# yeyupiaoling/PPASR

Measured on AMD Instinct MI355X. Metric: audio-seconds/s (RTF^-1) Conformer-streaming fbank, batch32 per GPU, ctc_greedy, higher is better.
Workload: dtype f32

## Files before the change

ppasr_amd/csrc/front_fused.hip:

```cpp
#include "conformer_kernels.h"
#include "launch.h"

namespace ppasr {

template <int MT>
__global__ __launch_bounds__(kThreads) void k_conv12(const float* __restrict__ feats, FrontW fw, float* __restrict__ out,
                                                     int T, int F, int Tp, int F2, int M, int m0, PadSkip ps,
                                                     const int* __restrict__ tile_tab) {
  constexpr int BM = 32 * MT, KC = 128, LD = KC + 4, G = KC / 8, NL = 2 * MT, STEP = G / NL, N_CHUNKS = 18;
  int r0 = m0 + blockIdx.x * BM, Mlim = M;
  if (tile_tab) {
    const int t = blockIdx.x, nb = tile_tab[0];
    const int* pre = tile_tab + 1;
    if (t >= pre[nb]) return;
    int lo = 0, hi = nb;
    while (hi - lo > 1) {
      const int mid = (lo + hi) >> 1;
      if (pre[mid] <= t) lo = mid;
      else hi = mid;
    }
    const int S = ps.Tp * ps.unit;
    r0 = lo * S + (t - pre[lo]) * BM;
    Mlim = min(M, (lo + 1) * S);
  } else if (pad_block_skippable(ps, r0, BM, M)) {
    return;
  }
  extern __shared__ __attribute__((aligned(16))) float smem[];
  float* xs = smem + 2 * BM * LD;
  const int tid = threadIdx.x, lane = lane_id(), wave = wave_id();
  constexpr int tile_stride = N_CHUNKS * G * 64;
  const f32x4* wbase = fw.conv2_w + (size_t)wave * tile_stride;
  BRing<1> ring;
  ring_prime(ring, wbase, 0);
  const int bt0 = r0 / F2, nbt = (min(r0 + BM, Mlim) - 1) / F2 - bt0 + 1;
  for (int idx = tid; idx < nbt * 7 * F; idx += kThreads) {
    const int p = idx / F, f = idx - p * F;
    const int btl = p / 7, fr = p - 7 * btl;
    const int bt = bt0 + btl, b = bt / Tp, tp = bt - b * Tp;
    const int t = min(4 * tp + fr, T - 1);
    xs[idx] = (feats[((size_t)b * T + t) * F + f] - fw.cmvn_mean[f]) * fw.cmvn_istd[f];
  }
  const int c4 = tid & 31, rbase = tid >> 5;
  uint32_t pb[MT];
#pragma unroll
  for (int i = 0; i < NL; ++i) {
    const int m = r0 + rbase + 16 * i;
    const int bt = m / F2, f2 = m - bt * F2;
    const uint32_t v = m < Mlim ? (uint32_t)((bt - bt0) * 7 * F + 4 * f2) : 0xffffu;
    pb[i >> 1] = (i & 1) ? (pb[i >> 1] | (v << 16)) : v;
  }
  auto pbase = [&](int i) { return (int)((i & 1) ? (pb[i >> 1] >> 16) : (pb[i >> 1] & 0xffffu)); };
  const int lds_off0 = rbase * LD + 4 * c4;
  f32x4 wv[9], bv;
  float xv[9];
  auto load_w = [&](int kc) {
    const int c = (kc & 1) * 128 + 4 * c4;
#pragma unroll
    for (int j = 0; j < 9; ++j) wv[j] = *reinterpret_cast<const f32x4*>(fw.conv1_w + j * 256 + c);
    bv = *reinterpret_cast<const f32x4*>(fw.conv1_b + c);
  };
  auto read_x = [&](int i, int toff) {
    const int o = pbase(i);
    const float* p = xs + (o == 0xffff ? 0 : o) + toff;
#pragma unroll
    for (int ii = 0; ii < 3; ++ii)
#pragma unroll
      for (int jj = 0; jj < 3; ++jj) xv[ii * 3 + jj] = p[ii * F + jj];
  };
  auto fma_row = [&](int i, float* buf) {
    f32x4 a = {0.f, 0.f, 0.f, 0.f};
#pragma unroll
    for (int j = 0; j < 9; ++j)
#pragma unroll
      for (int e = 0; e < 4; ++e) a[e] = fmaf(wv[j][e], xv[j], a[e]);
    a += bv;
#pragma unroll
    for (int e = 0; e < 4; ++e) a[e] = pbase(i) != 0xffff ? fmaxf(a[e], 0.f) : 0.f;
    *reinterpret_cast<f32x4*>(buf + lds_off0 + i * 16 * LD) = a;
  };
  auto tap_off = [&](int kc) {
    const int tap = kc >> 1, kh = tap / 3, kw = tap - 3 * kh;
    return 2 * kh * F + 2 * kw;
  };
  f32x16 acc[MT][1];
  acc_zero(acc);
  load_w(0);
  __syncthreads();
#pragma unroll
  for (int i = 0; i < NL; ++i) {
    read_x(i, 0);
    fma_row(i, smem);
  }
  __syncthreads();
  for (int kc = 0; kc < N_CHUNKS; ++kc) {
    float* cur = smem + (kc & 1) * BM * LD;
    float* nxt = smem + ((kc + 1) & 1) * BM * LD;
    const f32x4* seg = wbase + (size_t)kc * G * 64;
    if (kc + 1 < N_CHUNKS) {
      load_w(kc + 1);
      const int toff = tap_off(kc + 1);
      auto side = [&](int g) {
        const int i = g / STEP, ph = g - i * STEP;
        if (i < NL && ph == 0) read_x(i, toff);
        if (i < NL && ph == 1) fma_row(i, nxt);
      };
      rb_gemm<MT, 1, G, kPF, decltype(side)>(cur, LD, seg, 0, seg + G * 64, 0, ring, acc, side);
    } else {
      rb_gemm<MT, 1, G>(cur, LD, seg, 0, nullptr, 0, ring, acc);
    }
    __syncthreads();
  }
  const int col = wave * 32 + (lane & 31);
  const float b2 = fw.conv2_b[col];
#pragma unroll
  for (int mt = 0; mt < MT; ++mt)
#pragma unroll
    for (int r = 0; r < 16; ++r) {
      const int m = r0 + mt * 32 + acc_row(r, lane);
      const float v = fmaxf((acc[mt][0][r] + b2) * 1.0f, 0.f);
      if (m < Mlim) out[(size_t)m * 256 + col] = v;
    }
}

static size_t conv12_lds(int mt, int F, int F2) {
  const int bm = 32 * mt, nbt = (bm - 1) / F2 + 2;
  return ((size_t)2 * bm * 132 + (size_t)nbt * 7 * F) * sizeof(float);
}
bool conv12_supported(const FrontW& fw, int F, int F2) {
  return fw.conv2_k == 3 && fw.conv2_s == 2 && F2 >= 1 && conv12_lds(4, F, F2) <= 160 * 1024 &&
         (size_t)((127 / F2) + 2) * 7 * F < 0xffff;
}

void launch_tile_prefix(const PadSkip& ps, int B, int BM, int* tab, hipStream_t st);

void launch_conv12(const float* feats, const FrontW& fw, float* y2, int B, int T, int F, int Tp, int F2, hipStream_t st,
                   const PadSkip& ps_frames, int* tile_scratch) {
  PadSkip ps = ps_frames;
  ps.unit = F2;
  const int M = B * Tp * F2;
  constexpr int kCUs = 256;
  const int* no_tab = nullptr;
#define CONV12(MTA, GRID, M0, TAB)                                                                                      \
  PPASR_LAUNCH(k_conv12<MTA>, dim3(GRID), dim3(kThreads), conv12_lds(MTA, F, F2), st, feats, fw, y2, T, F, Tp, F2, M, M0, \
               ps, TAB)
  if (ps.lens && tile_scratch && M > 128 * kCUs) {
    launch_tile_prefix(ps, B, 128, tile_scratch, st);
    const int per_utt = (Tp * F2 + 127) / 128;
    CONV12(4, B * per_utt, 0, (const int*)tile_scratch);
    return;
  }
  const int tiles4 = (M + 127) / 128;
  const int full = (tiles4 / kCUs) * kCUs;
  const int rem_rows = M - full * 128;
  const int mt_rem = (rem_rows + 32 * kCUs - 1) / (32 * kCUs);
  if (full == 0) {
    const int mt = (M + 32 * kCUs - 1) / (32 * kCUs);
    if (mt <= 1) CONV12(1, (M + 31) / 32, 0, no_tab);
    else if (mt == 2) CONV12(2, (M + 63) / 64, 0, no_tab);
    else if (mt == 3) CONV12(3, (M + 95) / 96, 0, no_tab);
    else CONV12(4, (M + 127) / 128, 0, no_tab);
    return;
  }
  if (rem_rows <= 0 || mt_rem >= 4) {
    CONV12(4, tiles4, 0, no_tab);
    return;
  }
  CONV12(4, full, 0, no_tab);
  const int m0 = full * 128;
  if (mt_rem <= 1) CONV12(1, (rem_rows + 31) / 32, m0, no_tab);
  else if (mt_rem == 2) CONV12(2, (rem_rows + 63) / 64, m0, no_tab);
  else CONV12(3, (rem_rows + 95) / 96, m0, no_tab);
#undef CONV12
}

hipError_t configure_front_fused_kernels() {
  hipError_t e;
#define SET_LDS(fn)                                                                                              \
  e = hipFuncSetAttribute(reinterpret_cast<const void*>(fn), hipFuncAttributeMaxDynamicSharedMemorySize, 160 * 1024); \
  if (e != hipSuccess) return e;
  SET_LDS(k_conv12<1>);
  SET_LDS(k_conv12<2>);
  SET_LDS(k_conv12<3>);
  SET_LDS(k_conv12<4>);
#undef SET_LDS
  return hipSuccess;
}

}
```

Measured before the change: 54340.

## Compute conv1 with 32x32x2 f32 MFMA interleaved into conv2 GEMM

Replaces the scalar-FMA conv1 (9 taps times 4 channels per thread) with MFMA 32x32x2 f32 instructions over 5 k-steps. The work is spread across waves in 32-row tiles and interleaved into the conv2 GEMM side-slot schedule. The conv1 bias is staged in the LDS padding columns, and ReLU plus pad masking are applied with fmed3. The feature load is rewritten to be row-per-wave with hoisted CMVN constants and batched loads. The goal is to cut VALU cost of the on-the-fly conv1 recompute, at the price of more register pressure and a rearranged output layout.

After: 54700, median of 6. No clear change (+0.7%).

```diff
diff --git a/ppasr_amd/csrc/front_fused.hip b/ppasr_amd/csrc/front_fused.hip
--- a/ppasr_amd/csrc/front_fused.hip
+++ b/ppasr_amd/csrc/front_fused.hip
@@ -7,7 +7,9 @@
 __global__ __launch_bounds__(kThreads) void k_conv12(const float* __restrict__ feats, FrontW fw, float* __restrict__ out,
                                                      int T, int F, int Tp, int F2, int M, int m0, PadSkip ps,
                                                      const int* __restrict__ tile_tab) {
-  constexpr int BM = 32 * MT, KC = 128, LD = KC + 4, G = KC / 8, NL = 2 * MT, STEP = G / NL, N_CHUNKS = 18;
+  constexpr int BM = 32 * MT, KC = 128, LD = KC + 4, G = KC / 8, N_CHUNKS = 18;
+  constexpr int NT1 = (4 * MT + kWaves - 1) / kWaves;
+  static_assert(G == 16, "two conv1 tiles of 7 k-groups each per chunk");
   int r0 = m0 + blockIdx.x * BM, Mlim = M;
   if (tile_tab) {
     const int t = blockIdx.x, nb = tile_tab[0];
@@ -33,50 +35,83 @@
   BRing<1> ring;
   ring_prime(ring, wbase, 0);
   const int bt0 = r0 / F2, nbt = (min(r0 + BM, Mlim) - 1) / F2 - bt0 + 1;
-  for (int idx = tid; idx < nbt * 7 * F; idx += kThreads) {
-    const int p = idx / F, f = idx - p * F;
-    const int btl = p / 7, fr = p - 7 * btl;
-    const int bt = bt0 + btl, b = bt / Tp, tp = bt - b * Tp;
-    const int t = min(4 * tp + fr, T - 1);
-    xs[idx] = (feats[((size_t)b * T + t) * F + f] - fw.cmvn_mean[f]) * fw.cmvn_istd[f];
-  }
-  const int c4 = tid & 31, rbase = tid >> 5;
-  uint32_t pb[MT];
-#pragma unroll
-  for (int i = 0; i < NL; ++i) {
-    const int m = r0 + rbase + 16 * i;
+  {
+    const int nrow = nbt * 7, f0 = lane, f1 = lane + 64;
+    const float mu0 = f0 < F ? fw.cmvn_mean[f0] : 0.f, is0 = f0 < F ? fw.cmvn_istd[f0] : 0.f;
+    const float mu1 = f1 < F ? fw.cmvn_mean[f1] : 0.f, is1 = f1 < F ? fw.cmvn_istd[f1] : 0.f;
+    for (int pb = wave; pb < nrow; pb += 8 * kWaves) {
+      float v0[8], v1[8];
+#pragma unroll
+      for (int u = 0; u < 8; ++u) {
+        const int p = pb + u * kWaves;
+        v0[u] = v1[u] = 0.f;
+        if (p < nrow) {
+          const int btl = p / 7, fr = p - 7 * btl;
+          const int bt = bt0 + btl, b = bt / Tp, tp = bt - b * Tp;
+          const float* src = feats + ((size_t)b * T + min(4 * tp + fr, T - 1)) * F;
+          if (f0 < F) v0[u] = src[f0];
+          if (f1 < F) v1[u] = src[f1];
+        }
+      }
+#pragma unroll
+      for (int u = 0; u < 8; ++u) {
+        const int p = pb + u * kWaves;
+        if (p < nrow) {
+          if (f0 < F) xs[p * F + f0] = (v0[u] - mu0) * is0;
+          if (f1 < F) xs[p * F + f1] = (v1[u] - mu1) * is1;
+        }
+      }
+    }
+  }
+  if (tid < 256) smem[(tid >> 2) * LD + KC + (tid & 3)] = fw.conv1_b[tid];
+  const int h = lane >> 5, ct = wave & 3;
+  const int nt1 = (4 * MT) % kWaves == 0 ? NT1 : (4 * MT - wave + kWaves - 1) / kWaves;
+  int off[5];
+#pragma unroll
+  for (int s = 0; s < 5; ++s) {
+    const int j = min(2 * s + h, 8);
+    off[s] = (j / 3) * F + j % 3;
+  }
+  float w1[2][5];
+#pragma unroll
+  for (int par = 0; par < 2; ++par)
+#pragma unroll
+    for (int s = 0; s < 5; ++s) {
+      const int j = 2 * s + h;
+      w1[par][s] = j < 9 ? fw.conv1_w[j * 256 + par * 128 + ct * 32 + (lane & 31)] : 0.f;
+    }
+  int xo[NT1];
+  float hi[NT1];
+#pragma unroll
+  for (int i = 0; i < NT1; ++i) {
+    const int m = r0 + ((wave >> 2) + 2 * i) * 32 + (lane & 31);
     const int bt = m / F2, f2 = m - bt * F2;
-    const uint32_t v = m < Mlim ? (uint32_t)((bt - bt0) * 7 * F + 4 * f2) : 0xffffu;
-    pb[i >> 1] = (i & 1) ? (pb[i >> 1] | (v << 16)) : v;
-  }
-  auto pbase = [&](int i) { return (int)((i & 1) ? (pb[i >> 1] >> 16) : (pb[i >> 1] & 0xffffu)); };
-  const int lds_off0 = rbase * LD + 4 * c4;
-  f32x4 wv[9], bv;
-  float xv[9];
-  auto load_w = [&](int kc) {
-    const int c = (kc & 1) * 128 + 4 * c4;
-#pragma unroll
-    for (int j = 0; j < 9; ++j) wv[j] = *reinterpret_cast<const f32x4*>(fw.conv1_w + j * 256 + c);
-    bv = *reinterpret_cast<const f32x4*>(fw.conv1_b + c);
-  };
-  auto read_x = [&](int i, int toff) {
-    const int o = pbase(i);
-    const float* p = xs + (o == 0xffff ? 0 : o) + toff;
-#pragma unroll
-    for (int ii = 0; ii < 3; ++ii)
-#pragma unroll
-      for (int jj = 0; jj < 3; ++jj) xv[ii * 3 + jj] = p[ii * F + jj];
-  };
-  auto fma_row = [&](int i, float* buf) {
-    f32x4 a = {0.f, 0.f, 0.f, 0.f};
-#pragma unroll
-    for (int j = 0; j < 9; ++j)
-#pragma unroll
-      for (int e = 0; e < 4; ++e) a[e] = fmaf(wv[j][e], xv[j], a[e]);
-    a += bv;
-#pragma unroll
-    for (int e = 0; e < 4; ++e) a[e] = pbase(i) != 0xffff ? fmaxf(a[e], 0.f) : 0.f;
-    *reinterpret_cast<f32x4*>(buf + lds_off0 + i * 16 * LD) = a;
+    const bool ok = i < nt1 && m < Mlim;
+    xo[i] = ok ? (bt - bt0) * 7 * F + 4 * f2 : 0;
+    hi[i] = ok ? __builtin_inff() : 0.f;
+  }
+  f32x16 y1;
+  float xv[5];
+  auto c1_read = [&](int i, int toff) {
+    const float* p = xs + xo[i] + toff;
+#pragma unroll
+    for (int s = 0; s < 5; ++s) xv[s] = p[off[s]];
+    if (h) xv[4] = 0.f;
+  };
+  auto c1_mfma = [&](int s, int par) {
+    const float w = par ? w1[1][s] : w1[0][s];
+    y1 = __builtin_amdgcn_mfma_f32_32x32x2f32(w, xv[s], s == 0 ? f32x16{} : y1, 0, 0, 0);
+  };
+  auto c1_store = [&](int i, float* buf, int par) {
+    const float* bq = smem + (par * 32 + ct * 8 + h) * LD + KC;
+    float* dst = buf + (((wave >> 2) + 2 * i) * 32 + (lane & 31)) * LD + ct * 32 + 4 * h;
+#pragma unroll
+    for (int q = 0; q < 4; ++q) {
+      f32x4 v = f32x4{y1[4 * q], y1[4 * q + 1], y1[4 * q + 2], y1[4 * q + 3]} + *reinterpret_cast<const f32x4*>(bq + 2 * q * LD);
+#pragma unroll
+      for (int e = 0; e < 4; ++e) v[e] = __builtin_amdgcn_fmed3f(v[e], 0.f, hi[i]);
+      *reinterpret_cast<f32x4*>(dst + 8 * q) = v;
+    }
   };
   auto tap_off = [&](int kc) {
     const int tap = kc >> 1, kh = tap / 3, kw = tap - 3 * kh;
@@ -84,12 +119,15 @@
   };
   f32x16 acc[MT][1];
   acc_zero(acc);
-  load_w(0);
   __syncthreads();
 #pragma unroll
-  for (int i = 0; i < NL; ++i) {
-    read_x(i, 0);
-    fma_row(i, smem);
+  for (int i = 0; i < NT1; ++i) {
+    if (i < nt1) {
+      c1_read(i, 0);
+#pragma unroll
+      for (int s = 0; s < 5; ++s) c1_mfma(s, 0);
+      c1_store(i, smem, 0);
+    }
   }
   __syncthreads();
   for (int kc = 0; kc < N_CHUNKS; ++kc) {
@@ -97,12 +135,14 @@
     float* nxt = smem + ((kc + 1) & 1) * BM * LD;
     const f32x4* seg = wbase + (size_t)kc * G * 64;
     if (kc + 1 < N_CHUNKS) {
-      load_w(kc + 1);
-      const int toff = tap_off(kc + 1);
+      const int toff = tap_off(kc + 1), par = (kc + 1) & 1;
       auto side = [&](int g) {
-        const int i = g / STEP, ph = g - i * STEP;
-        if (i < NL && ph == 0) read_x(i, toff);
-        if (i < NL && ph == 1) fma_row(i, nxt);
+        const int i = g >> 3, ph = g & 7;
+        if (i < nt1) {
+          if (ph == 0) c1_read(i, toff);
+          else if (ph <= 5) c1_mfma(ph - 1, par);
+          else if (ph == 6) c1_store(i, nxt, par);
+        }
       };
       rb_gemm<MT, 1, G, kPF, decltype(side)>(cur, LD, seg, 0, seg + G * 64, 0, ring, acc, side);
     } else {
@@ -110,13 +150,14 @@
     }
     __syncthreads();
   }
-  const int col = wave * 32 + (lane & 31);
+  const int lane_e = (int)__builtin_amdgcn_mbcnt_hi(~0u, __builtin_amdgcn_mbcnt_lo(~0u, 0u));
+  const int col = wave * 32 + (lane_e & 31);
   const float b2 = fw.conv2_b[col];
 #pragma unroll
   for (int mt = 0; mt < MT; ++mt)
 #pragma unroll
     for (int r = 0; r < 16; ++r) {
-      const int m = r0 + mt * 32 + acc_row(r, lane);
+      const int m = r0 + mt * 32 + acc_row(r, lane_e);
       const float v = fmaxf((acc[mt][0][r] + b2) * 1.0f, 0.f);
       if (m < Mlim) out[(size_t)m * 256 + col] = v;
     }
@@ -127,8 +168,7 @@
   return ((size_t)2 * bm * 132 + (size_t)nbt * 7 * F) * sizeof(float);
 }
 bool conv12_supported(const FrontW& fw, int F, int F2) {
-  return fw.conv2_k == 3 && fw.conv2_s == 2 && F2 >= 1 && conv12_lds(4, F, F2) <= 160 * 1024 &&
-         (size_t)((127 / F2) + 2) * 7 * F < 0xffff;
+  return fw.conv2_k == 3 && fw.conv2_s == 2 && F2 >= 1 && F <= 128 && conv12_lds(4, F, F2) <= 160 * 1024;
 }
 
 void launch_tile_prefix(const PadSkip& ps, int B, int BM, int* tab, hipStream_t st);
```
